# mynameisfiber/baton

Hardware: NVIDIA H100
Metric: federated local samples/sec (whole box), ResNet-18 FedAvg, synthetic non-IID 32x32 shards (higher is better)
Workload: dtype bf16

## Files before the change

baton_b200/csrc/bindings.cpp:

```cpp
#include <ATen/cuda/CUDAContext.h>
#include <c10/cuda/CUDAGuard.h>
#include <torch/extension.h>

#include <optional>
#include <vector>

#include "launch.h"

namespace {

inline cudaStream_t cur_stream() { return at::cuda::getCurrentCUDAStream().stream(); }
inline void check(int rc, const char* what) {
  TORCH_CHECK(rc == 0, "baton_b200::", what, " failed with code ", rc,
              rc > 0 ? std::string(" (") + cudaGetErrorString(static_cast<cudaError_t>(rc)) + ")" : std::string());
}
inline const void* cptr(const at::Tensor& t) { return t.data_ptr(); }
inline void* ptr(at::Tensor& t) { return t.data_ptr(); }
template <class T>
inline T* opt_ptr(const std::optional<at::Tensor>& t) {
  return (t.has_value() && t->defined()) ? reinterpret_cast<T*>(t->data_ptr()) : nullptr;
}
#define CHECK_CUDA(x) TORCH_CHECK((x).is_cuda(), #x " must be a CUDA tensor")

inline const float* prox_anchor(const std::optional<at::Tensor>& anchor, int64_t numel, const at::Tensor& hyper) {
// ... 233 lines not shown
  const int64_t c = src.size(3);
  const int64_t rows = src.size(0) * ((src.size(1) - 1) / stride + 1) * ((src.size(2) - 1) / stride + 1);
  TORCH_CHECK(rows > 0 && out.numel() % rows == 0, "conv_halo: out must hold [N*Ho*Wo, Nout] elements");
  const int64_t nout = out.numel() / rows;
  TORCH_CHECK(w.numel() == (dgrad ? c * 9 * nout : nout * 9 * c), "conv_halo: w must be [Cout, 9*Cin]");
  TORCH_CHECK(dgrad ? !col_stats.has_value()
                    : (!col_stats.has_value() || (col_stats->scalar_type() == at::kFloat && col_stats->numel() >= 2 * nout)),
              "conv_halo: col_stats is a [2 Cout] fp32 buffer of the forward");
  const c10::cuda::CUDAGuard guard(src.device());
  const int rc = b200_conv_halo(cptr(src), cptr(w), ptr(out), static_cast<int>(src.size(0)), static_cast<int>(src.size(1)),
                                static_cast<int>(src.size(2)), static_cast<int>(c), static_cast<int>(nout),
                                static_cast<int>(stride), dgrad ? 1 : 0, static_cast<int>(mc), opt_ptr<float>(col_stats),
                                cur_stream());
  if (rc == -2) return false;
  check(rc, "conv_halo");
  return true;
}
bool conv_igemm_dgrad_s2(const at::Tensor& dy, const at::Tensor& w, at::Tensor dx, int64_t kh, int64_t kw,
                         const std::vector<int64_t>& ntaps, const std::vector<int64_t>& taps, int64_t force_bn) {
  CHECK_CUDA(dy); CHECK_CUDA(w); CHECK_CUDA(dx);
  TORCH_CHECK(dy.scalar_type() == at::kBFloat16 && w.scalar_type() == at::kBFloat16 && dx.scalar_type() == at::kBFloat16 &&
              dy.dim() == 4 && dx.dim() == 4 && dy.is_contiguous() && w.is_contiguous() && dx.is_contiguous());
  TORCH_CHECK(ntaps.size() == 4 && taps.size() == 16, "conv_igemm_dgrad_s2: 4 classes x 4 taps");
  int nt[4], tw[16];
  for (int i = 0; i < 4; ++i) nt[i] = static_cast<int>(ntaps[i]);
  for (int i = 0; i < 16; ++i) tw[i] = static_cast<int>(taps[i]);
  const c10::cuda::CUDAGuard guard(dy.device());
  const int rc = b200_conv_igemm_dgrad_s2(cptr(dy), cptr(w), ptr(dx), static_cast<int>(dx.size(0)),
                                          static_cast<int>(dx.size(1)), static_cast<int>(dx.size(2)),
                                          static_cast<int>(dx.size(3)), static_cast<int>(dy.size(3)), static_cast<int>(kh),
// ... 1160 lines not shown
  m.doc() = "baton_b200 sm_90a kernels";
  m.attr("MAX_RANKS") = B200_MAX_RANKS;
  m.def("gemm", &gemm);
  m.def("trace_set", &trace_set);
  m.def("attention_fwd", &attention_fwd);
  m.def("attention_bwd", &attention_bwd);
  m.def("bn_bwd_cluster", &bn_bwd_cluster);
  m.def("gn_fwd", &gn_fwd);
  m.def("gn_bwd", &gn_bwd);
  m.def("im2col_tma_probe", &im2col_tma_probe);
  m.def("conv_igemm_fwd", &conv_igemm_fwd);
  m.def("conv_igemm_wgrad", &conv_igemm_wgrad);
  m.def("conv_igemm_dgrad", &conv_igemm_dgrad);
  m.def("conv_igemm_dgrad_s2", &conv_igemm_dgrad_s2);
  m.def("conv_halo", &conv_halo);
  m.def("gemm_batched", &gemm_batched);
  m.def("gemm_fp8", &gemm_fp8);
  m.def("quant_mx_rows", &quant_mx_rows);
  m.def("quant_mx_cols", &quant_mx_cols);
  m.def("fused_sgd", &fused_sgd);
  m.def("fused_sgd_segments", &fused_sgd_segments);
  m.def("grad_norm_clip", &grad_norm_clip);
  m.attr("GRAD_NORM_WORK_WORDS") = B200_GRAD_NORM_WORK_WORDS;
  m.def("weighted_sum", &weighted_sum);
  m.def("fold_client", &fold_client);
  m.def("scaffold_corr", &scaffold_corr);
  m.def("scaffold_dc", &scaffold_dc);
  m.def("cast", &cast);
  m.def("gather_rows", &gather_rows);
  m.def("gather_augment", &gather_augment);
// ... 59 lines not shown
```

baton_b200/csrc/conv_halo.cu:

```cuda
#define B200_TU_TAG 12
#include "ptx.cuh"
#include "epilogue.cuh"
#include "launch.h"
#include "pdl.cuh"

namespace b200 {

constexpr int HALO_BM = 64;
constexpr int HALO_BN = 64;
constexpr int HALO_TAPS = 9;
constexpr int HALO_THREADS = 256;
constexpr int HALO_CONSUMERS = 128;
constexpr int HALO_SLOT_BYTES = 64 * 64 * 2;
constexpr int HALO_PART_PITCH = HALO_BN + 4;
constexpr int HALO_MAX_SMEM = 227 * 1024;

struct HaloParams {
  int M, N;
  int Ho, Wo;
  __nv_bfloat16* D;
  float* col_stats;
  int ncol;
  int mc;
  int halo_bytes;
};

__host__ __device__ constexpr int halo_barriers(int k_tiles) { return (1 + k_tiles + 15) / 16 * 16; }

__host__ __device__ constexpr int halo_fixed_bytes(int k_tiles) {
  return k_tiles * HALO_SLOT_BYTES + halo_barriers(k_tiles) * 8 + 4 * HALO_BN * 4 + 1024;
}

template <bool DGRAD, int CB, int STRIDE>
__global__ void __launch_bounds__(HALO_THREADS, 1)
conv_halo_kernel(const __grid_constant__ CUtensorMap tmX, const __grid_constant__ CUtensorMap tmW, const HaloParams p) {
  constexpr int KT = HALO_TAPS * CB;
  extern __shared__ __align__(1024) uint8_t smem_raw[];
  uint8_t* smem = reinterpret_cast<uint8_t*>((reinterpret_cast<uintptr_t>(smem_raw) + 1023) & ~uintptr_t(1023));
  uint8_t* halo = smem;
  uint8_t* bslot = smem + CB * p.halo_bytes;
  uint64_t* bar = reinterpret_cast<uint64_t*>(bslot + KT * HALO_SLOT_BYTES);
  float* cstat = reinterpret_cast<float*>(bar + halo_barriers(KT));

  griddep_launch_dependents();
  const int warp = threadIdx.x >> 5;
  const int m0 = blockIdx.y * HALO_BM;
  const int n0 = blockIdx.x * HALO_BN;
  const int hw = p.Ho * p.Wo;
  const int hp = STRIDE * (p.Ho - 1) + 3, wp = STRIDE * (p.Wo - 1) + 3;

  if (warp == 0 && elect_one()) {
    tma_prefetch_desc(&tmX);
    tma_prefetch_desc(&tmW);
    for (int i = 0; i < 1 + KT; ++i) mbar_init(&bar[i], 1);
    fence_barrier_init();
  }
  __syncthreads();
  if (p.mc > 1) cluster_sync_all();
  griddep_wait();

  if (warp == 0) {
    if (elect_one()) {
      const int imgs = HALO_BM / hw;
      mbar_expect_tx(&bar[0], CB * imgs * hp * wp * 128);
#pragma unroll
      for (int cb = 0; cb < CB; ++cb) tma_load_4d(halo + cb * p.halo_bytes, &tmX, &bar[0], 64 * cb, -1, -1, m0 / hw);
      const int rows = 64 / p.mc;
      const int rank = p.mc > 1 ? static_cast<int>(cluster_ctarank()) : 0;
      const uint16_t mask = static_cast<uint16_t>((1u << p.mc) - 1);
#pragma unroll 1
      for (int kt = 0; kt < KT; ++kt) {
        const int tap = kt / CB, cb = kt - tap * CB;
        mbar_expect_tx(&bar[1 + kt], HALO_SLOT_BYTES);
        uint8_t* dst = bslot + kt * HALO_SLOT_BYTES + rank * rows * 128;
        const int c0 = DGRAD ? (HALO_TAPS - 1 - tap) * p.ncol + n0 : kt * 64;
        const int c1 = DGRAD ? cb * 64 + rank * rows : n0 + rank * rows;
        if (p.mc > 1)
          tma_load_2d_mc(dst, &tmW, &bar[1 + kt], c0, c1, mask);
        else
          tma_load_2d(dst, &tmW, &bar[1 + kt], c0, c1);
      }
    }
  } else if (warp >= 4) {
    const int ew = warp - 4;
    const int lane = static_cast<int>(lane_id());
    const int m = 16 * ew + (lane & 15);
    const int img = m / hw, rem = m - img * hw;
    const int oi = rem / p.Wo, oj = rem - oi * p.Wo;
    const int hrow0 = (img * hp + STRIDE * oi) * wp + STRIDE * oj;
    const uint32_t halo_a = smem_u32(halo);
    const int half = lane >> 4;
    auto load_a = [&](uint32_t (&a)[4][4], int kt) {
      const int tap = kt / CB, cb = kt - tap * CB;
      const int r = tap / 3, s = tap - 3 * r;
      const int hrow = hrow0 + r * wp + s;
      const uint32_t row_addr = halo_a + static_cast<uint32_t>(cb * p.halo_bytes + hrow * 128);
#pragma unroll
      for (int kk = 0; kk < 4; ++kk) ldmatrix_x4(a[kk], row_addr + ((((2 * kk + half) ^ hrow) & 7) << 4));
    };

    float acc[32];
#pragma unroll
    for (int j = 0; j < 32; ++j) acc[j] = 0.f;
    uint32_t a[2][4][4];
    mbar_wait(&bar[0], 0);
    load_a(a[0], 0);
#pragma unroll
    for (int kt = 0; kt < KT; ++kt) {
      mbar_wait(&bar[1 + kt], 0);
      const uint32_t sb = smem_u32(bslot + kt * HALO_SLOT_BYTES);
      wgmma_fence();
#pragma unroll
      for (int kk = 0; kk < 4; ++kk) {
        const uint64_t bd = DGRAD ? gmma_desc_sw128(sb + kk * 2048, 8192, 1024) : gmma_desc_sw128(sb + kk * 32, 16, 1024);
        wgmma_bf16_n64_rs<DGRAD ? 1 : 0>(acc, a[kt & 1][kk], bd, 1u);
      }
      wgmma_commit();
      if (kt + 1 < KT) {
        wgmma_wait<1>();
        load_a(a[(kt + 1) & 1], kt + 1);
      }
    }
    wgmma_wait<0>();
    wgmma_fence_operands(acc);
    if (threadIdx.x == 128) TRACE_POINT();

    named_bar_sync(1, HALO_CONSUMERS);
    float* part = reinterpret_cast<float*>(smem);
    wg_store_acc<HALO_BN>(acc, part, HALO_PART_PITCH, 0);
    named_bar_sync(1, HALO_CONSUMERS);
    const int q = ew & 1;
    const int c = (ew >> 1) * 32;
    const int lrow = q * 32 + lane;
    const int row = m0 + lrow;
    const int col0 = n0 + c;
    float* sstat = cstat + q * 2 * HALO_BN;
    const bool want_stats = p.col_stats != nullptr;
    if (col0 >= p.N) {
      if (want_stats) { sstat[c + lane] = 0.f; sstat[HALO_BN + c + lane] = 0.f; }
    } else {
      uint32_t r[32];
      acc_ld_row32(part + lrow * HALO_PART_PITCH + c, r);
      float v[32];
#pragma unroll
      for (int j = 0; j < 32; ++j) v[j] = __uint_as_float(r[j]);
      if (want_stats) stage_col_stats(sstat, HALO_BN, c, v);
      if (row < p.M) {
        __nv_bfloat16* d = p.D + static_cast<size_t>(row) * p.N + col0;
        if (col0 + 32 <= p.N && (p.N % 8) == 0) {
#pragma unroll
          for (int j = 0; j < 32; j += 8) {
            uint4 o;
            o.x = pack_bf16x2(v[j], v[j + 1]);
            o.y = pack_bf16x2(v[j + 2], v[j + 3]);
            o.z = pack_bf16x2(v[j + 4], v[j + 5]);
            o.w = pack_bf16x2(v[j + 6], v[j + 7]);
            *reinterpret_cast<uint4*>(d + j) = o;
          }
        } else {
          _Pragma("unroll") for (int j = 0; j < 32; ++j) if (col0 + j < p.N) d[j] = __float2bfloat16_rn(v[j]);
        }
      }
    }
    if (want_stats) {
      named_bar_sync(1, HALO_CONSUMERS);
      for (int i = threadIdx.x - 128; i < 2 * HALO_BN; i += HALO_CONSUMERS) {
        const int col = i < HALO_BN ? i : i - HALO_BN;
        if (n0 + col < p.N)
          atomicAdd(p.col_stats + (i < HALO_BN ? 0 : p.N) + n0 + col,
                    cstat[i] + cstat[2 * HALO_BN + i]);
      }
    }
  }
}

template <auto KERNEL>
static int launch_halo(const CUtensorMap& tx, const CUtensorMap& tw, const HaloParams& p, dim3 grid, int smem,
                       cudaStream_t stream) {
  static bool configured = false;
  if (!configured) {
    cudaError_t e = cudaFuncSetAttribute(KERNEL, cudaFuncAttributeMaxDynamicSharedMemorySize,
                                         HALO_MAX_SMEM);
    if (e != cudaSuccess) return static_cast<int>(e);
    configured = true;
  }
// ... 11 lines not shown
  }
  if (p.mc > 1) {
    attr[na].id = cudaLaunchAttributeClusterDimension;
    attr[na].val.clusterDim.x = 1;
    attr[na].val.clusterDim.y = p.mc;
    attr[na].val.clusterDim.z = 1;
    ++na;
  }
  cfg.attrs = attr;
  cfg.numAttrs = na;
  cudaError_t le = cudaLaunchKernelEx(&cfg, KERNEL, tx, tw, p);
  if (le != cudaSuccess) return static_cast<int>(le);
  return static_cast<int>(cudaGetLastError());
}

}

extern "C" int b200_encode_map2_bf16(void* map, const void* base, long long rows, long long cols, long long ld,
                                     int box_cols, int box_rows);
extern "C" int b200_encode_map4_box_bf16(void* map, const void* base, const long long* dims,
                                         const long long* stride_bytes, const int* box);

extern "C" int b200_conv_halo(const void* src, const void* w, void* out, int N, int H, int W, int C, int Nout,
                              int stride, int dgrad, int mc, float* col_stats, cudaStream_t stream) {
  using namespace b200;
  const bool s1c64 = stride == 1 && C == 64, s1c128 = stride == 1 && C == 128, s2c64 = stride == 2 && C == 64 && !dgrad;
  if (!s1c64 && !s1c128 && !s2c64) return -2;
  const int Ho = (H - 1) / stride + 1, Wo = (W - 1) / stride + 1;
  const long long M = static_cast<long long>(N) * Ho * Wo;
  if (M <= 0 || Nout <= 0) return 0;
  const int hw = Ho * Wo;
  const long long m_tiles = (M + HALO_BM - 1) / HALO_BM;
  const int hp = stride * (Ho - 1) + 3, wp = stride * (Wo - 1) + 3;
  if (H <= 0 || W <= 0 || HALO_BM % hw != 0 || hp > 256 || wp > 256 || M > (1ll << 30) || Nout % 8 != 0 ||
      (dgrad && Nout % 64 != 0) || (mc != 1 && mc != 2 && mc != 4 && mc != 8) || m_tiles % mc != 0 ||
      (reinterpret_cast<uintptr_t>(src) & 15) || (reinterpret_cast<uintptr_t>(w) & 15) ||
      (reinterpret_cast<uintptr_t>(out) & 15))
    return -2;
  const int imgs = HALO_BM / hw;
  const int cb = C / 64;
  const int halo_bytes = (imgs * hp * wp * 128 + 1023) / 1024 * 1024;
  const int smem = cb * halo_bytes + halo_fixed_bytes(HALO_TAPS * cb);
  if (smem > HALO_MAX_SMEM) return -2;
  CUtensorMap tx, tw;
  const long long dims[4] = {C, W, H, N};
  const long long strides[3] = {static_cast<long long>(C) * 2, static_cast<long long>(W) * C * 2,
                                static_cast<long long>(H) * W * C * 2};
  const int box[4] = {64, wp, hp, imgs};
  int rc = b200_encode_map4_box_bf16(&tx, src, dims, strides, box);
  if (rc) return rc;
  const long long wrows = dgrad ? C : Nout, wcols = dgrad ? 9ll * Nout : 9ll * C;
  rc = b200_encode_map2_bf16(&tw, w, wrows, wcols, wcols, 64, 64 / mc);
  if (rc) return rc;
  HaloParams p;
  p.M = static_cast<int>(M); p.N = Nout; p.Ho = Ho; p.Wo = Wo; p.D = reinterpret_cast<__nv_bfloat16*>(out);
  p.col_stats = col_stats; p.ncol = Nout; p.mc = mc; p.halo_bytes = halo_bytes;
  dim3 grid((Nout + HALO_BN - 1) / HALO_BN, static_cast<unsigned>(m_tiles), 1);
  if (s2c64) return launch_halo<conv_halo_kernel<false, 1, 2>>(tx, tw, p, grid, smem, stream);
  if (s1c64)
    return dgrad ? launch_halo<conv_halo_kernel<true, 1, 1>>(tx, tw, p, grid, smem, stream)
                 : launch_halo<conv_halo_kernel<false, 1, 1>>(tx, tw, p, grid, smem, stream);
  return dgrad ? launch_halo<conv_halo_kernel<true, 2, 1>>(tx, tw, p, grid, smem, stream)
               : launch_halo<conv_halo_kernel<false, 2, 1>>(tx, tw, p, grid, smem, stream);
}

B200_TRACE_REGISTER(conv_halo)
```

baton_b200/csrc/gemm_wgmma.cu:

```cuda
#define B200_TU_TAG 1
#include "ptx.cuh"
#include "epilogue.cuh"
#include "launch.h"
#include "pdl.cuh"
#include "sgd.cuh"

namespace b200 {

constexpr int BM = 128;
constexpr int BK = 64;
constexpr int WG_K = 16;
constexpr int GEMM_THREADS = 384;
constexpr int CONSUMER_WARPS = 8;
constexpr int CONSUMER_THREADS = 32 * CONSUMER_WARPS;
constexpr int MAX_STAGES = 8;
constexpr int S2_MAX_TAPS = 4;

struct GemmParams {
  int M, N, K;
  void* D;
  long long ldd;
  const float* bias;
  int out_fp32;
  int act;
// ... 962 lines not shown
    cudaFree(nullptr);
    ctx_bound = true;
  }
  static EncodeTiledFn fn = nullptr;
  if (fn == nullptr) {
    void* ptr = nullptr;
    cudaDriverEntryPointQueryResult qres;
    cudaError_t e = cudaGetDriverEntryPoint("cuTensorMapEncodeTiled", &ptr, cudaEnableDefault, &qres);
    if (e != cudaSuccess || qres != cudaDriverEntryPointSuccess || ptr == nullptr) return nullptr;
    fn = reinterpret_cast<EncodeTiledFn>(ptr);
  }
  return fn;
}

static int make_map(CUtensorMap* map, const void* base, long long rows, long long cols, long long ld, int box_cols,
                    int box_rows) {
  EncodeTiledFn fn = get_encode_fn();
  if (fn == nullptr) return -1;
  cuuint64_t gdim[2] = {static_cast<cuuint64_t>(cols), static_cast<cuuint64_t>(rows)};
  cuuint64_t gstr[1] = {static_cast<cuuint64_t>(ld) * 2};
  cuuint32_t box[2] = {static_cast<cuuint32_t>(box_cols), static_cast<cuuint32_t>(box_rows)};
  cuuint32_t estr[2] = {1, 1};
  CUresult r = fn(map, CU_TENSOR_MAP_DATA_TYPE_BFLOAT16, 2, const_cast<void*>(base), gdim, gstr, box, estr,
                  CU_TENSOR_MAP_INTERLEAVE_NONE, CU_TENSOR_MAP_SWIZZLE_128B, CU_TENSOR_MAP_L2_PROMOTION_L2_256B,
                  CU_TENSOR_MAP_FLOAT_OOB_FILL_NONE);
  return r == CUDA_SUCCESS ? 0 : static_cast<int>(r);
}

static int make_map4(CUtensorMap* map, const void* base, long long rows, long long cols, long long ld, long long inner,
                     long long s_inner, long long outer, long long s_outer, int box_cols, int box_rows) {
  EncodeTiledFn fn = get_encode_fn();
  if (fn == nullptr) return -1;
  cuuint64_t gdim[4] = {static_cast<cuuint64_t>(cols), static_cast<cuuint64_t>(rows), static_cast<cuuint64_t>(inner),
                        static_cast<cuuint64_t>(outer)};
  cuuint64_t gstr[3] = {static_cast<cuuint64_t>(ld) * 2, static_cast<cuuint64_t>(s_inner) * 2,
                        static_cast<cuuint64_t>(s_outer) * 2};
  cuuint32_t box[4] = {static_cast<cuuint32_t>(box_cols), static_cast<cuuint32_t>(box_rows), 1, 1};
  cuuint32_t estr[4] = {1, 1, 1, 1};
  CUresult r = fn(map, CU_TENSOR_MAP_DATA_TYPE_BFLOAT16, 4, const_cast<void*>(base), gdim, gstr, box, estr,
// ... 115 lines not shown
    ++na;
  }
  cfg.attrs = attr;
  cfg.numAttrs = na;
  cudaError_t le = p.cluster_k > 1 ? cudaLaunchKernelEx(&cfg, gemm_bf16_splitk_kernel<BN, true, CONV, AFFINE>, ta, tb, p)
                                   : cudaLaunchKernelEx(&cfg, gemm_bf16_splitk_kernel<BN, false, CONV, AFFINE>, ta, tb, p);
  if (le != cudaSuccess) return static_cast<int>(le);
  return static_cast<int>(cudaGetLastError());
}

}

extern "C" int b200_encode_map2_bf16(void* map, const void* base, long long rows, long long cols, long long ld,
                                     int box_cols, int box_rows) {
  return b200::make_map(reinterpret_cast<CUtensorMap*>(map), base, rows, cols, ld, box_cols, box_rows);
}
extern "C" int b200_encode_map4_bf16(void* map, const void* base, long long rows, long long cols, long long ld,
                                     long long inner, long long s_inner, long long outer, long long s_outer,
                                     int box_cols, int box_rows) {
  return b200::make_map4(reinterpret_cast<CUtensorMap*>(map), base, rows, cols, ld, inner, s_inner, outer, s_outer,
                         box_cols, box_rows);
}
extern "C" int b200_encode_map4_box_bf16(void* map, const void* base, const long long* dims, const long long* stride_bytes,
                                         const int* box) {
  b200::EncodeTiledFn fn = b200::get_encode_fn();
  if (fn == nullptr) return -1;
  cuuint64_t gdim[4], gstr[3];
  cuuint32_t bx[4], estr[4] = {1, 1, 1, 1};
  for (int i = 0; i < 4; ++i) {
    gdim[i] = static_cast<cuuint64_t>(dims[i]);
// ... 333 lines not shown
```

baton_b200/csrc/launch.h:

```cpp
#pragma once
#include <cuda_runtime.h>
#include <stdint.h>

#define B200_MAX_RANKS 16

extern "C" {

struct B200SgdEpilogue {
  float* theta;
  void* theta_bf16;
  float* mom;
  const float* hyper;
  int nesterov;
  const float* anchor;
  const float* corr;
  float* v;
};
#define B200_SGD_EPILOGUE_DECLINED (-6)

struct B200AffineEpilogue {
  const float* scale;
  const float* shift;
  const void* residual;
  long long ldr;
// ... 19 lines not shown
                            const B200Dropout* drop, cudaStream_t stream);
int b200_attention_drop_bwd(const void* qkv, const void* dout, const void* probs, void* dqkv, int B, int S, int H, int dh,
                            float scale, const B200Dropout* drop, cudaStream_t stream);
int b200_conv_igemm_fwd(const void* x, const void* w, void* y, int N, int H, int W, int Cin, int Cout, int KH, int KW,
                        int stride, int pad, int Ho, int Wo, int cluster_k, int force_bn, float* col_stats,
                        const B200AffineEpilogue* affine, cudaStream_t stream);
int b200_conv_igemm_dgrad(const void* dy, const void* w, void* dx, int N, int H, int W, int Cin, int Cout, int KH, int KW,
                          int pad, int Ho, int Wo, int cluster_k, int force_bn, cudaStream_t stream);
int b200_conv_igemm_dgrad_s2(const void* dy, const void* w, void* dx, int N, int H, int W, int Cin, int Cout, int KH,
                             int KW, int Ho, int Wo, const int* ntaps, const int* taps, int force_bn, cudaStream_t stream);
int b200_conv_igemm_wgrad(const void* dy, const void* x, float* dw, int N, int H, int W, int Cin, int Cout, int KH, int KW,
                          int stride, int pad, int Ho, int Wo, int split_k, int force_bn, const B200SgdEpilogue* sgd,
                          cudaStream_t stream);
int b200_conv_halo(const void* src, const void* w, void* out, int N, int H, int W, int C, int Nout, int stride,
                   int dgrad, int mc, float* col_stats, cudaStream_t stream);
int b200_im2col_tma_probe(const void* x, void* col, int N, int H, int W, int C, int KH, int KW, int stride, int pad,
                          int Ho, int Wo, cudaStream_t stream);
int b200_gemm_fp8(const void* a, const void* b, void* d, const float* bias, const void* sfa, const void* sfb, int M, int N,
                  int K, long long lda, long long ldb, long long ldd, int out_fp32, int act, int split_k, int accumulate,
                  float alpha, cudaStream_t stream);
int b200_quant_mx_rows(const void* x, void* q, void* sf, long long R, int C, long long ld_in, int Cp, cudaStream_t stream);
int b200_quant_mx_cols(const void* x, void* q, void* sf, long long R, int C, long long ld_in, long long Rp,
                       cudaStream_t stream);
int b200_gemm_simt(const void* a, const void* b, void* d, const float* bias, int M, int N, int K, long long lda,
                   long long ldb, long long ldd, int a_mn, int b_mn, int out_fp32, int act, int accumulate,
                   float alpha, cudaStream_t stream);

int b200_fused_sgd(float* w, float* g, float* mom, void* w_bf16, long long n, const float* hyper, int zero_grad,
                   int nesterov, const unsigned long long* wire_slot, const float* pack_global,
                   const float* pack_scale, long long n_pack, int wire_fp32, const float* prox_anchor,
// ... 240 lines not shown
```

baton_b200/csrc/ptx.cuh:

```cuda
#pragma once
#include <cuda.h>
#include <cuda_bf16.h>
#include <cuda_runtime.h>
#include <stdint.h>

namespace b200 {

__device__ __forceinline__ uint32_t smem_u32(const void* p) {
  return static_cast<uint32_t>(__cvta_generic_to_shared(p));
}
__device__ __forceinline__ uint32_t lane_id() {
  uint32_t l;
  asm volatile("mov.u32 %0, %%laneid;" : "=r"(l));
  return l;
}
__device__ __forceinline__ bool elect_one() {
  uint32_t pred;
  asm volatile(
      "{\n\t.reg .pred p;\n\t"
      "elect.sync _|p, 0xffffffff;\n\t"
      "selp.u32 %0, 1, 0, p;\n\t}"
      : "=r"(pred));
  return pred != 0;
}
// ... 78 lines not shown
}
template <int NR>
__device__ __forceinline__ void wgmma_fence_operands(float (&d)[NR]) {
#pragma unroll
  for (int i = 0; i < NR; ++i) asm volatile("" : "+f"(d[i])::"memory");
}

__device__ __forceinline__ uint64_t gmma_desc_sw128(uint32_t smem_addr, uint32_t lbo_bytes, uint32_t sbo_bytes) {
  uint64_t d = 0;
  d |= static_cast<uint64_t>((smem_addr & 0x3FFFF) >> 4);
  d |= static_cast<uint64_t>((lbo_bytes >> 4) & 0x3FFF) << 16;
  d |= static_cast<uint64_t>((sbo_bytes >> 4) & 0x3FFF) << 32;
  d |= static_cast<uint64_t>(1) << 62;
  return d;
}

template <int TA, int TB>
__device__ __forceinline__ void wgmma_bf16_n64(float (&d)[32], uint64_t da, uint64_t db, uint32_t scale_d) {
  asm volatile(
      "{\n\t.reg .pred p;\n\tsetp.ne.b32 p, %34, 0;\n\t"
      "wgmma.mma_async.sync.aligned.m64n64k16.f32.bf16.bf16 "
      "{"
      "%0, %1, %2, %3, %4, %5, %6, %7, %8, %9, %10, %11, %12, %13, %14, %15, "
      "%16, %17, %18, %19, %20, %21, %22, %23, %24, %25, %26, %27, %28, %29, %30, %31"
      "}, %32, %33, p, 1, 1, %35, %36;\n\t}"
      : "+f"(d[0]), "+f"(d[1]), "+f"(d[2]), "+f"(d[3]), "+f"(d[4]), "+f"(d[5]), "+f"(d[6]), "+f"(d[7]),
        "+f"(d[8]), "+f"(d[9]), "+f"(d[10]), "+f"(d[11]), "+f"(d[12]), "+f"(d[13]), "+f"(d[14]), "+f"(d[15]),
        "+f"(d[16]), "+f"(d[17]), "+f"(d[18]), "+f"(d[19]), "+f"(d[20]), "+f"(d[21]), "+f"(d[22]), "+f"(d[23]),
        "+f"(d[24]), "+f"(d[25]), "+f"(d[26]), "+f"(d[27]), "+f"(d[28]), "+f"(d[29]), "+f"(d[30]), "+f"(d[31])
      : "l"(da), "l"(db), "r"(scale_d), "n"(TA), "n"(TB));
// ... 20 lines not shown
      : "l"(da), "l"(db), "r"(scale_d), "n"(TA), "n"(TB));
}
template <int TB>
__device__ __forceinline__ void wgmma_bf16_n64_rs(float (&d)[32], const uint32_t (&a)[4], uint64_t db, uint32_t scale_d) {
  asm volatile(
      "{\n\t.reg .pred p;\n\tsetp.ne.b32 p, %37, 0;\n\t"
      "wgmma.mma_async.sync.aligned.m64n64k16.f32.bf16.bf16 "
      "{"
      "%0, %1, %2, %3, %4, %5, %6, %7, %8, %9, %10, %11, %12, %13, %14, %15, "
      "%16, %17, %18, %19, %20, %21, %22, %23, %24, %25, %26, %27, %28, %29, %30, %31"
      "}, {%32, %33, %34, %35}, %36, p, 1, 1, %38;\n\t}"
      : "+f"(d[0]), "+f"(d[1]), "+f"(d[2]), "+f"(d[3]), "+f"(d[4]), "+f"(d[5]), "+f"(d[6]), "+f"(d[7]),
        "+f"(d[8]), "+f"(d[9]), "+f"(d[10]), "+f"(d[11]), "+f"(d[12]), "+f"(d[13]), "+f"(d[14]), "+f"(d[15]),
        "+f"(d[16]), "+f"(d[17]), "+f"(d[18]), "+f"(d[19]), "+f"(d[20]), "+f"(d[21]), "+f"(d[22]), "+f"(d[23]),
        "+f"(d[24]), "+f"(d[25]), "+f"(d[26]), "+f"(d[27]), "+f"(d[28]), "+f"(d[29]), "+f"(d[30]), "+f"(d[31])
      : "r"(a[0]), "r"(a[1]), "r"(a[2]), "r"(a[3]), "l"(db), "r"(scale_d), "n"(TB));
}
__device__ __forceinline__ void ldmatrix_x4(uint32_t (&r)[4], uint32_t smem_addr) {
  asm volatile("ldmatrix.sync.aligned.m8n8.x4.shared.b16 {%0, %1, %2, %3}, [%4];"
               : "=r"(r[0]), "=r"(r[1]), "=r"(r[2]), "=r"(r[3])
               : "r"(smem_addr)
               : "memory");
}
__device__ __forceinline__ void wgmma_e4m3_n64(float (&d)[32], uint64_t da, uint64_t db, uint32_t scale_d) {
  asm volatile(
      "{\n\t.reg .pred p;\n\tsetp.ne.b32 p, %34, 0;\n\t"
      "wgmma.mma_async.sync.aligned.m64n64k32.f32.e4m3.e4m3 "
      "{"
      "%0, %1, %2, %3, %4, %5, %6, %7, %8, %9, %10, %11, %12, %13, %14, %15, "
      "%16, %17, %18, %19, %20, %21, %22, %23, %24, %25, %26, %27, %28, %29, %30, %31"
// ... 140 lines not shown
```

baton_b200/ops/functional.py:

```python
from __future__ import annotations

import collections
import functools
from typing import List, Optional, Sequence, Tuple

import torch

from ._ext import load

BF16 = torch.bfloat16
NUM_SMS = 132


def _pitch(t: torch.Tensor) -> int:
    assert t.dim() == 2 and (t.stride(1) == 1 or t.shape[1] == 1), "GEMM operand must have unit inner stride"
    return t.stride(0) if t.shape[0] > 1 else max(t.stride(0), t.shape[1])


def _tma_ok(t: torch.Tensor) -> bool:
    return t.dtype == BF16 and _pitch(t) % 8 == 0 and t.data_ptr() % 16 == 0


def pick_bn(M: int, N: int) -> int:
    m_tiles = (M + 127) // 128
# ... 412 lines not shown

def halo_eligible(kh: int, kw: int, stride: int, pad: int, c: int, h: int, w: int,
                  affine: Optional[dict] = None, dgrad: bool = False) -> bool:
    if kh != 3 or kw != 3 or pad != 1 or (stride, c) not in _HALO_FORMS or (dgrad and stride != 1):
        return False
    hw = conv_out_size(h, 3, stride, 1) * conv_out_size(w, 3, stride, 1)
    return (hw <= HALO_BM and HALO_BM % hw == 0 and affine is None and
            halo_smem_bytes(h, w, c, stride) <= _HALO_MAX_SMEM)


def halo_cluster(m_rows: int) -> int:
    tiles = (m_rows + HALO_BM - 1) // HALO_BM
    return 4 if tiles % 4 == 0 else 2 if tiles % 2 == 0 else 1


def _conv_path(path: Optional[str], eligible: bool) -> str:
    if path is None:
        return "halo" if eligible else "im2col"
    if path not in ("halo", "im2col"):
        raise ValueError("path must be None, 'halo' or 'im2col', not {!r}".format(path))
    if path == "halo" and not eligible:
        raise ValueError("the halo kernel does not take this convolution (see halo_eligible)")
    return path


def conv_igemm_fwd(x: torch.Tensor, w2d: torch.Tensor, kh: int, kw: int, stride: int, pad: int,
                   col_stats: Optional[torch.Tensor] = None, affine: Optional[dict] = None,
                   cluster_k: Optional[int] = None, force_bn: int = 0,
                   out: Optional[torch.Tensor] = None, path: Optional[str] = None,
                   mc: Optional[int] = None) -> Optional[torch.Tensor]:
    n, h, w, c = x.shape
    cout = w2d.shape[0]
    if c % 64 or w2d.shape[1] != kh * kw * c or not x.is_contiguous() or not w2d.is_contiguous():
        return None
    ho, wo = conv_out_size(h, kh, stride, pad), conv_out_size(w, kw, stride, pad)
    M, K = n * ho * wo, kh * kw * c
    halo = halo_eligible(kh, kw, stride, pad, c, h, w, affine) and cout % 8 == 0
    if _conv_path(path, halo) == "halo":
        y = out if out is not None else torch.empty((M, cout), dtype=BF16, device=x.device)
        if not load().conv_halo(x, w2d, y, stride, False, mc or halo_cluster(M), col_stats):
            raise RuntimeError("conv_halo declined a convolution halo_eligible admits")
        return y
    bn = force_bn or pick_bn(M, cout)
    if cluster_k is None:
        cluster_k = pick_cluster_k(M, cout, K, bn)
    y = out if out is not None else torch.empty((M, cout), dtype=BF16, device=x.device)
    af = affine or {}
    ok = load().conv_igemm_fwd(x, w2d, y, kh, kw, stride, pad, ho, wo, cluster_k, bn, col_stats, af.get("scale"),
                               af.get("shift"), af.get("residual"), bool(af.get("relu", False)))
    return y if ok else None


S2_MAX_TAPS = 4


def conv_s2_dgrad_taps(kh: int, kw: int, pad: int, ho: int, wo: int) -> Optional[List[List[Tuple[int, int, int]]]]:
# ... 14 lines not shown
                    if dp < ho and dq < wo:
                        taps.append((r * kw + s, dp, dq))
            if len(taps) > S2_MAX_TAPS:
                return None
            classes.append(taps)
    return classes


def conv_igemm_dgrad(dy: torch.Tensor, w2d: torch.Tensor, in_shape, kh: int, kw: int, pad: int, stride: int = 1,
                     out: Optional[torch.Tensor] = None, path: Optional[str] = None,
                     mc: Optional[int] = None, cluster_k: Optional[int] = None) -> Optional[torch.Tensor]:
    n, h, w, c = in_shape
    cout = dy.shape[-1]
    if c % 64 or cout % 64 or w2d.shape[1] != kh * kw * c or not dy.is_contiguous() or not w2d.is_contiguous():
        return None
    if _conv_path(path, halo_eligible(kh, kw, stride, pad, cout, h, w, dgrad=True)) == "halo":
        dx = out if out is not None else torch.empty((n, h, w, c), dtype=BF16, device=dy.device)
        if not load().conv_halo(dy, w2d, dx, 1, True, mc or halo_cluster(n * h * w), None):
            raise RuntimeError("conv_halo declined a convolution halo_eligible admits")
        return dx
    if stride == 1:
        M, K = n * h * w, kh * kw * cout
        bn = pick_bn(M, c)
        dx = out if out is not None else torch.empty((n, h, w, c), dtype=BF16, device=dy.device)
        if cluster_k is None:
            cluster_k = pick_cluster_k(M, c, K, bn)
        ok = load().conv_igemm_dgrad(dy, w2d, dx, kh, kw, pad, cluster_k, bn)
        return dx if ok else None
    if stride != 2:
        return None
    ho, wo = dy.shape[1], dy.shape[2]
    classes = conv_s2_dgrad_taps(kh, kw, pad, ho, wo)
    if classes is None:
        return None
# ... 220 lines not shown
```

Before: 223,900.

## Add small-feature-map conv kernel with whole-image tiles and 32-wide columns

Adds a conv_smallmap path for 3x3 pad-1 convolutions on small maps (stride-1 C=256 and stride-2 C=128), used in both forward and dgrad. The kernel stages whole images in shared memory with no TMA padding halo and reads a zero line in place of out-of-image taps. It uses n32 wgmma tiles with 64B-swizzled weight loads, which yields more CTAs on the deep ResNet layers, where M is small and the im2col GEMM path underfills the GPU. The cost is more kernel variants, extra per-tap bounds checks, and halved N per MMA.

```diff
diff --git a/baton_b200/csrc/bindings.cpp b/baton_b200/csrc/bindings.cpp
--- a/baton_b200/csrc/bindings.cpp
+++ b/baton_b200/csrc/bindings.cpp
@@ -271,6 +271,29 @@
                                 cur_stream());
   if (rc == -2) return false;
   check(rc, "conv_halo");
+  return true;
+}
+bool conv_smallmap(const at::Tensor& src, const at::Tensor& w, at::Tensor out, int64_t stride, bool dgrad, int64_t mc,
+                   int64_t bn, const std::optional<at::Tensor>& col_stats) {
+  CHECK_CUDA(src); CHECK_CUDA(w); CHECK_CUDA(out);
+  TORCH_CHECK(src.scalar_type() == at::kBFloat16 && w.scalar_type() == at::kBFloat16 && out.scalar_type() == at::kBFloat16 &&
+              src.dim() == 4 && src.is_contiguous() && w.is_contiguous() && out.is_contiguous());
+  TORCH_CHECK(stride == 1 || stride == 2, "conv_smallmap: stride 1 or 2");
+  const int64_t c = src.size(3);
+  const int64_t rows = src.size(0) * ((src.size(1) - 1) / stride + 1) * ((src.size(2) - 1) / stride + 1);
+  TORCH_CHECK(rows > 0 && out.numel() % rows == 0, "conv_smallmap: out must hold [N*Ho*Wo, Nout] elements");
+  const int64_t nout = out.numel() / rows;
+  TORCH_CHECK(w.numel() == (dgrad ? c * 9 * nout : nout * 9 * c), "conv_smallmap: w must be [Cout, 9*Cin]");
+  TORCH_CHECK(dgrad ? !col_stats.has_value()
+                    : (!col_stats.has_value() || (col_stats->scalar_type() == at::kFloat && col_stats->numel() >= 2 * nout)),
+              "conv_smallmap: col_stats is a [2 Cout] fp32 buffer of the forward");
+  const c10::cuda::CUDAGuard guard(src.device());
+  const int rc = b200_conv_smallmap(cptr(src), cptr(w), ptr(out), static_cast<int>(src.size(0)),
+                                    static_cast<int>(src.size(1)), static_cast<int>(src.size(2)), static_cast<int>(c),
+                                    static_cast<int>(nout), static_cast<int>(stride), dgrad ? 1 : 0, static_cast<int>(mc),
+                                    static_cast<int>(bn), opt_ptr<float>(col_stats), cur_stream());
+  if (rc == -2) return false;
+  check(rc, "conv_smallmap");
   return true;
 }
 bool conv_igemm_dgrad_s2(const at::Tensor& dy, const at::Tensor& w, at::Tensor dx, int64_t kh, int64_t kw,
@@ -1461,6 +1484,7 @@
   m.def("conv_igemm_dgrad", &conv_igemm_dgrad);
   m.def("conv_igemm_dgrad_s2", &conv_igemm_dgrad_s2);
   m.def("conv_halo", &conv_halo);
+  m.def("conv_smallmap", &conv_smallmap);
   m.def("gemm_batched", &gemm_batched);
   m.def("gemm_fp8", &gemm_fp8);
   m.def("quant_mx_rows", &quant_mx_rows);
diff --git a/baton_b200/csrc/conv_halo.cu b/baton_b200/csrc/conv_halo.cu
--- a/baton_b200/csrc/conv_halo.cu
+++ b/baton_b200/csrc/conv_halo.cu
@@ -11,9 +11,8 @@
 constexpr int HALO_TAPS = 9;
 constexpr int HALO_THREADS = 256;
 constexpr int HALO_CONSUMERS = 128;
-constexpr int HALO_SLOT_BYTES = 64 * 64 * 2;
-constexpr int HALO_PART_PITCH = HALO_BN + 4;
 constexpr int HALO_MAX_SMEM = 227 * 1024;
+constexpr int HALO_ZERO_BYTES = 128;
 
 struct HaloParams {
   int M, N;
@@ -23,31 +22,39 @@
   int ncol;
   int mc;
   int halo_bytes;
+  int bh, bw;
 };
 
 __host__ __device__ constexpr int halo_barriers(int k_tiles) { return (1 + k_tiles + 15) / 16 * 16; }
 
-__host__ __device__ constexpr int halo_fixed_bytes(int k_tiles) {
-  return k_tiles * HALO_SLOT_BYTES + halo_barriers(k_tiles) * 8 + 4 * HALO_BN * 4 + 1024;
-}
-
-template <bool DGRAD, int CB, int STRIDE>
+__host__ __device__ constexpr int halo_slot_bytes(int bn) { return bn * 64 * 2; }
+
+__host__ __device__ constexpr int halo_fixed_bytes(int k_tiles, int bn = HALO_BN, bool img = false) {
+  return k_tiles * halo_slot_bytes(bn) + halo_barriers(k_tiles) * 8 + 4 * bn * 4 + (img ? HALO_ZERO_BYTES : 0) + 1024;
+}
+
+template <bool DGRAD, int CB, int STRIDE, int BN = HALO_BN, bool IMG = false>
 __global__ void __launch_bounds__(HALO_THREADS, 1)
 conv_halo_kernel(const __grid_constant__ CUtensorMap tmX, const __grid_constant__ CUtensorMap tmW, const HaloParams p) {
+  static_assert(BN == 32 || BN == 64, "conv_halo_kernel: 32 or 64 columns");
   constexpr int KT = HALO_TAPS * CB;
+  constexpr int SLOT = halo_slot_bytes(BN);
+  constexpr int PITCH = BN + 4;
+  constexpr int ORIGIN = IMG ? 0 : -1;
   extern __shared__ __align__(1024) uint8_t smem_raw[];
   uint8_t* smem = reinterpret_cast<uint8_t*>((reinterpret_cast<uintptr_t>(smem_raw) + 1023) & ~uintptr_t(1023));
   uint8_t* halo = smem;
   uint8_t* bslot = smem + CB * p.halo_bytes;
-  uint64_t* bar = reinterpret_cast<uint64_t*>(bslot + KT * HALO_SLOT_BYTES);
+  uint64_t* bar = reinterpret_cast<uint64_t*>(bslot + KT * SLOT);
   float* cstat = reinterpret_cast<float*>(bar + halo_barriers(KT));
+  uint8_t* zline = reinterpret_cast<uint8_t*>(cstat + 4 * BN);
 
   griddep_launch_dependents();
   const int warp = threadIdx.x >> 5;
   const int m0 = blockIdx.y * HALO_BM;
-  const int n0 = blockIdx.x * HALO_BN;
+  const int n0 = blockIdx.x * BN;
   const int hw = p.Ho * p.Wo;
-  const int hp = STRIDE * (p.Ho - 1) + 3, wp = STRIDE * (p.Wo - 1) + 3;
+  const int hp = p.bh, wp = p.bw;
 
   if (warp == 0 && elect_one()) {
     tma_prefetch_desc(&tmX);
@@ -64,15 +71,19 @@
       const int imgs = HALO_BM / hw;
       mbar_expect_tx(&bar[0], CB * imgs * hp * wp * 128);
 #pragma unroll
-      for (int cb = 0; cb < CB; ++cb) tma_load_4d(halo + cb * p.halo_bytes, &tmX, &bar[0], 64 * cb, -1, -1, m0 / hw);
-      const int rows = 64 / p.mc;
+      for (int cb = 0; cb < CB; ++cb)
+        tma_load_4d(halo + cb * p.halo_bytes, &tmX, &bar[0], 64 * cb, ORIGIN, ORIGIN, m0 / hw);
+      constexpr int SROWS = DGRAD ? 64 : BN;
+      constexpr int RB = SLOT / SROWS;
+      const int rows = max(SROWS / p.mc, 8);
       const int rank = p.mc > 1 ? static_cast<int>(cluster_ctarank()) : 0;
       const uint16_t mask = static_cast<uint16_t>((1u << p.mc) - 1);
 #pragma unroll 1
       for (int kt = 0; kt < KT; ++kt) {
         const int tap = kt / CB, cb = kt - tap * CB;
-        mbar_expect_tx(&bar[1 + kt], HALO_SLOT_BYTES);
-        uint8_t* dst = bslot + kt * HALO_SLOT_BYTES + rank * rows * 128;
+        mbar_expect_tx(&bar[1 + kt], SLOT);
+        if (rank * rows >= SROWS) continue;
+        uint8_t* dst = bslot + kt * SLOT + rank * rows * RB;
         const int c0 = DGRAD ? (HALO_TAPS - 1 - tap) * p.ncol + n0 : kt * 64;
         const int c1 = DGRAD ? cb * 64 + rank * rows : n0 + rank * rows;
         if (p.mc > 1)
@@ -87,33 +98,53 @@
     const int m = 16 * ew + (lane & 15);
     const int img = m / hw, rem = m - img * hw;
     const int oi = rem / p.Wo, oj = rem - oi * p.Wo;
-    const int hrow0 = (img * hp + STRIDE * oi) * wp + STRIDE * oj;
+    const int y0 = STRIDE * oi - 1 - ORIGIN, x0 = STRIDE * oj - 1 - ORIGIN;
+    const int hrow0 = (img * hp + y0) * wp + x0;
     const uint32_t halo_a = smem_u32(halo);
     const int half = lane >> 4;
     auto load_a = [&](uint32_t (&a)[4][4], int kt) {
       const int tap = kt / CB, cb = kt - tap * CB;
       const int r = tap / 3, s = tap - 3 * r;
       const int hrow = hrow0 + r * wp + s;
-      const uint32_t row_addr = halo_a + static_cast<uint32_t>(cb * p.halo_bytes + hrow * 128);
+      uint32_t row_addr = halo_a + static_cast<uint32_t>(cb * p.halo_bytes + hrow * 128);
+      if constexpr (IMG) {
+        const int y = y0 + r, x = x0 + s;
+        if (y < 0 || y >= hp || x < 0 || x >= wp) row_addr = smem_u32(zline);
+      }
 #pragma unroll
       for (int kk = 0; kk < 4; ++kk) ldmatrix_x4(a[kk], row_addr + ((((2 * kk + half) ^ hrow) & 7) << 4));
     };
 
-    float acc[32];
-#pragma unroll
-    for (int j = 0; j < 32; ++j) acc[j] = 0.f;
+    float acc[BN / 2];
+#pragma unroll
+    for (int j = 0; j < BN / 2; ++j) acc[j] = 0.f;
     uint32_t a[2][4][4];
+    if constexpr (IMG) {
+      if (threadIdx.x < 128 + HALO_ZERO_BYTES / 16) reinterpret_cast<uint4*>(zline)[threadIdx.x - 128] = make_uint4(0, 0, 0, 0);
+      named_bar_sync(1, HALO_CONSUMERS);
+    }
     mbar_wait(&bar[0], 0);
+    if (threadIdx.x == 128) TRACE_POINT();
     load_a(a[0], 0);
 #pragma unroll
     for (int kt = 0; kt < KT; ++kt) {
       mbar_wait(&bar[1 + kt], 0);
-      const uint32_t sb = smem_u32(bslot + kt * HALO_SLOT_BYTES);
+      if (threadIdx.x == 128 && (kt == 0 || kt == KT - 1)) TRACE_POINT();
+      const uint32_t sb = smem_u32(bslot + kt * SLOT);
       wgmma_fence();
 #pragma unroll
       for (int kk = 0; kk < 4; ++kk) {
-        const uint64_t bd = DGRAD ? gmma_desc_sw128(sb + kk * 2048, 8192, 1024) : gmma_desc_sw128(sb + kk * 32, 16, 1024);
-        wgmma_bf16_n64_rs<DGRAD ? 1 : 0>(acc, a[kt & 1][kk], bd, 1u);
+        uint64_t bd;
+        if constexpr (!DGRAD)
+          bd = gmma_desc_sw128(sb + kk * 32, 16, 1024);
+        else if constexpr (BN == 64)
+          bd = gmma_desc_sw128(sb + kk * 2048, 8192, 1024);
+        else
+          bd = gmma_desc_sw64(sb + kk * 1024, 4096, 512);
+        if constexpr (BN == 64)
+          wgmma_bf16_n64_rs<DGRAD ? 1 : 0>(acc, a[kt & 1][kk], bd, 1u);
+        else
+          wgmma_bf16_n32_rs<DGRAD ? 1 : 0>(acc, a[kt & 1][kk], bd, 1u);
       }
       wgmma_commit();
       if (kt + 1 < KT) {
@@ -127,24 +158,25 @@
 
     named_bar_sync(1, HALO_CONSUMERS);
     float* part = reinterpret_cast<float*>(smem);
-    wg_store_acc<HALO_BN>(acc, part, HALO_PART_PITCH, 0);
+    wg_store_acc<BN>(acc, part, PITCH, 0);
     named_bar_sync(1, HALO_CONSUMERS);
     const int q = ew & 1;
     const int c = (ew >> 1) * 32;
     const int lrow = q * 32 + lane;
     const int row = m0 + lrow;
     const int col0 = n0 + c;
-    float* sstat = cstat + q * 2 * HALO_BN;
+    float* sstat = cstat + q * 2 * BN;
     const bool want_stats = p.col_stats != nullptr;
-    if (col0 >= p.N) {
-      if (want_stats) { sstat[c + lane] = 0.f; sstat[HALO_BN + c + lane] = 0.f; }
+    if (c >= BN) {
+    } else if (col0 >= p.N) {
+      if (want_stats) { sstat[c + lane] = 0.f; sstat[BN + c + lane] = 0.f; }
     } else {
       uint32_t r[32];
-      acc_ld_row32(part + lrow * HALO_PART_PITCH + c, r);
+      acc_ld_row32(part + lrow * PITCH + c, r);
       float v[32];
 #pragma unroll
       for (int j = 0; j < 32; ++j) v[j] = __uint_as_float(r[j]);
-      if (want_stats) stage_col_stats(sstat, HALO_BN, c, v);
+      if (want_stats) stage_col_stats(sstat, BN, c, v);
       if (row < p.M) {
         __nv_bfloat16* d = p.D + static_cast<size_t>(row) * p.N + col0;
         if (col0 + 32 <= p.N && (p.N % 8) == 0) {
@@ -164,11 +196,11 @@
     }
     if (want_stats) {
       named_bar_sync(1, HALO_CONSUMERS);
-      for (int i = threadIdx.x - 128; i < 2 * HALO_BN; i += HALO_CONSUMERS) {
-        const int col = i < HALO_BN ? i : i - HALO_BN;
+      for (int i = threadIdx.x - 128; i < 2 * BN; i += HALO_CONSUMERS) {
+        const int col = i < BN ? i : i - BN;
         if (n0 + col < p.N)
-          atomicAdd(p.col_stats + (i < HALO_BN ? 0 : p.N) + n0 + col,
-                    cstat[i] + cstat[2 * HALO_BN + i]);
+          atomicAdd(p.col_stats + (i < BN ? 0 : p.N) + n0 + col,
+                    cstat[i] + cstat[2 * BN + i]);
       }
     }
   }
@@ -210,48 +242,72 @@
   return static_cast<int>(cudaGetLastError());
 }
 
+static int conv_tiled_setup(const void* src, const void* w, void* out, int N, int H, int W, int C, int Nout, int stride,
+                            int dgrad, int mc, int bn, bool img, float* col_stats, CUtensorMap* tx, CUtensorMap* tw,
+                            HaloParams* p, dim3* grid, int* smem);
+
 }
 
 extern "C" int b200_encode_map2_bf16(void* map, const void* base, long long rows, long long cols, long long ld,
                                      int box_cols, int box_rows);
+extern "C" int b200_encode_map2_sw64_bf16(void* map, const void* base, long long rows, long long cols, long long ld,
+                                          int box_cols, int box_rows);
 extern "C" int b200_encode_map4_box_bf16(void* map, const void* base, const long long* dims,
                                          const long long* stride_bytes, const int* box);
+
+namespace b200 {
+
+static int conv_tiled_setup(const void* src, const void* w, void* out, int N, int H, int W, int C, int Nout, int stride,
+                            int dgrad, int mc, int bn, bool img, float* col_stats, CUtensorMap* tx, CUtensorMap* tw,
+                            HaloParams* p, dim3* grid, int* smem) {
+  const int Ho = (H - 1) / stride + 1, Wo = (W - 1) / stride + 1;
+  const long long M = static_cast<long long>(N) * Ho * Wo;
+  if (M <= 0 || Nout <= 0) return 1;
+  const int hw = Ho * Wo;
+  const long long m_tiles = (M + HALO_BM - 1) / HALO_BM;
+  const int bh = img ? H : stride * (Ho - 1) + 3, bw = img ? W : stride * (Wo - 1) + 3;
+  if (H <= 0 || W <= 0 || HALO_BM % hw != 0 || bh > 256 || bw > 256 || M > (1ll << 30) || Nout % 8 != 0 ||
+      ((dgrad || img) && Nout % bn != 0) || (mc != 1 && mc != 2 && mc != 4 && mc != 8) || m_tiles % mc != 0 ||
+      (reinterpret_cast<uintptr_t>(src) & 15) || (reinterpret_cast<uintptr_t>(w) & 15) ||
+      (reinterpret_cast<uintptr_t>(out) & 15))
+    return -2;
+  const int imgs = HALO_BM / hw;
+  const int cb = C / 64;
+  const int box_bytes = (imgs * bh * bw * 128 + 1023) / 1024 * 1024;
+  *smem = cb * box_bytes + halo_fixed_bytes(HALO_TAPS * cb, bn, img);
+  if (*smem > HALO_MAX_SMEM) return -2;
+  const long long dims[4] = {C, W, H, N};
+  const long long strides[3] = {static_cast<long long>(C) * 2, static_cast<long long>(W) * C * 2,
+                                static_cast<long long>(H) * W * C * 2};
+  const int box[4] = {64, bw, bh, imgs};
+  int rc = b200_encode_map4_box_bf16(tx, src, dims, strides, box);
+  if (rc) return rc;
+  const long long wrows = dgrad ? C : Nout, wcols = dgrad ? 9ll * Nout : 9ll * C;
+  const int srows = dgrad ? 64 : bn;
+  const int rows = srows / mc > 8 ? srows / mc : 8;
+  rc = dgrad && bn == 32 ? b200_encode_map2_sw64_bf16(tw, w, wrows, wcols, wcols, bn, rows)
+                         : b200_encode_map2_bf16(tw, w, wrows, wcols, wcols, dgrad ? bn : 64, rows);
+  if (rc) return rc;
+  p->M = static_cast<int>(M); p->N = Nout; p->Ho = Ho; p->Wo = Wo; p->D = reinterpret_cast<__nv_bfloat16*>(out);
+  p->col_stats = col_stats; p->ncol = Nout; p->mc = mc; p->halo_bytes = box_bytes; p->bh = bh; p->bw = bw;
+  *grid = dim3((Nout + bn - 1) / bn, static_cast<unsigned>(m_tiles), 1);
+  return 0;
+}
+
+}
 
 extern "C" int b200_conv_halo(const void* src, const void* w, void* out, int N, int H, int W, int C, int Nout,
                               int stride, int dgrad, int mc, float* col_stats, cudaStream_t stream) {
   using namespace b200;
   const bool s1c64 = stride == 1 && C == 64, s1c128 = stride == 1 && C == 128, s2c64 = stride == 2 && C == 64 && !dgrad;
   if (!s1c64 && !s1c128 && !s2c64) return -2;
-  const int Ho = (H - 1) / stride + 1, Wo = (W - 1) / stride + 1;
-  const long long M = static_cast<long long>(N) * Ho * Wo;
-  if (M <= 0 || Nout <= 0) return 0;
-  const int hw = Ho * Wo;
-  const long long m_tiles = (M + HALO_BM - 1) / HALO_BM;
-  const int hp = stride * (Ho - 1) + 3, wp = stride * (Wo - 1) + 3;
-  if (H <= 0 || W <= 0 || HALO_BM % hw != 0 || hp > 256 || wp > 256 || M > (1ll << 30) || Nout % 8 != 0 ||
-      (dgrad && Nout % 64 != 0) || (mc != 1 && mc != 2 && mc != 4 && mc != 8) || m_tiles % mc != 0 ||
-      (reinterpret_cast<uintptr_t>(src) & 15) || (reinterpret_cast<uintptr_t>(w) & 15) ||
-      (reinterpret_cast<uintptr_t>(out) & 15))
-    return -2;
-  const int imgs = HALO_BM / hw;
-  const int cb = C / 64;
-  const int halo_bytes = (imgs * hp * wp * 128 + 1023) / 1024 * 1024;
-  const int smem = cb * halo_bytes + halo_fixed_bytes(HALO_TAPS * cb);
-  if (smem > HALO_MAX_SMEM) return -2;
   CUtensorMap tx, tw;
-  const long long dims[4] = {C, W, H, N};
-  const long long strides[3] = {static_cast<long long>(C) * 2, static_cast<long long>(W) * C * 2,
-                                static_cast<long long>(H) * W * C * 2};
-  const int box[4] = {64, wp, hp, imgs};
-  int rc = b200_encode_map4_box_bf16(&tx, src, dims, strides, box);
-  if (rc) return rc;
-  const long long wrows = dgrad ? C : Nout, wcols = dgrad ? 9ll * Nout : 9ll * C;
-  rc = b200_encode_map2_bf16(&tw, w, wrows, wcols, wcols, 64, 64 / mc);
-  if (rc) return rc;
   HaloParams p;
-  p.M = static_cast<int>(M); p.N = Nout; p.Ho = Ho; p.Wo = Wo; p.D = reinterpret_cast<__nv_bfloat16*>(out);
-  p.col_stats = col_stats; p.ncol = Nout; p.mc = mc; p.halo_bytes = halo_bytes;
-  dim3 grid((Nout + HALO_BN - 1) / HALO_BN, static_cast<unsigned>(m_tiles), 1);
+  dim3 grid;
+  int smem = 0;
+  const int rc = conv_tiled_setup(src, w, out, N, H, W, C, Nout, stride, dgrad, mc, HALO_BN, false, col_stats, &tx, &tw,
+                                  &p, &grid, &smem);
+  if (rc) return rc == 1 ? 0 : rc;
   if (s2c64) return launch_halo<conv_halo_kernel<false, 1, 2>>(tx, tw, p, grid, smem, stream);
   if (s1c64)
     return dgrad ? launch_halo<conv_halo_kernel<true, 1, 1>>(tx, tw, p, grid, smem, stream)
@@ -260,4 +316,24 @@
                : launch_halo<conv_halo_kernel<false, 2, 1>>(tx, tw, p, grid, smem, stream);
 }
 
+extern "C" int b200_conv_smallmap(const void* src, const void* w, void* out, int N, int H, int W, int C, int Nout,
+                                  int stride, int dgrad, int mc, int bn, float* col_stats, cudaStream_t stream) {
+  using namespace b200;
+  const bool s1c256 = stride == 1 && C == 256 && bn == 32;
+  const bool s2c128 = stride == 2 && C == 128 && !dgrad && (bn == 32 || bn == 64);
+  if (!s1c256 && !s2c128) return -2;
+  CUtensorMap tx, tw;
+  HaloParams p;
+  dim3 grid;
+  int smem = 0;
+  const int rc = conv_tiled_setup(src, w, out, N, H, W, C, Nout, stride, dgrad, mc, bn, true, col_stats, &tx, &tw, &p,
+                                  &grid, &smem);
+  if (rc) return rc == 1 ? 0 : rc;
+  if (s2c128)
+    return bn == 32 ? launch_halo<conv_halo_kernel<false, 2, 2, 32, true>>(tx, tw, p, grid, smem, stream)
+                    : launch_halo<conv_halo_kernel<false, 2, 2, 64, true>>(tx, tw, p, grid, smem, stream);
+  return dgrad ? launch_halo<conv_halo_kernel<true, 4, 1, 32, true>>(tx, tw, p, grid, smem, stream)
+               : launch_halo<conv_halo_kernel<false, 4, 1, 32, true>>(tx, tw, p, grid, smem, stream);
+}
+
 B200_TRACE_REGISTER(conv_halo)
diff --git a/baton_b200/csrc/gemm_wgmma.cu b/baton_b200/csrc/gemm_wgmma.cu
--- a/baton_b200/csrc/gemm_wgmma.cu
+++ b/baton_b200/csrc/gemm_wgmma.cu
@@ -1000,7 +1000,7 @@
 }
 
 static int make_map(CUtensorMap* map, const void* base, long long rows, long long cols, long long ld, int box_cols,
-                    int box_rows) {
+                    int box_rows, CUtensorMapSwizzle swizzle = CU_TENSOR_MAP_SWIZZLE_128B) {
   EncodeTiledFn fn = get_encode_fn();
   if (fn == nullptr) return -1;
   cuuint64_t gdim[2] = {static_cast<cuuint64_t>(cols), static_cast<cuuint64_t>(rows)};
@@ -1008,7 +1008,7 @@
   cuuint32_t box[2] = {static_cast<cuuint32_t>(box_cols), static_cast<cuuint32_t>(box_rows)};
   cuuint32_t estr[2] = {1, 1};
   CUresult r = fn(map, CU_TENSOR_MAP_DATA_TYPE_BFLOAT16, 2, const_cast<void*>(base), gdim, gstr, box, estr,
-                  CU_TENSOR_MAP_INTERLEAVE_NONE, CU_TENSOR_MAP_SWIZZLE_128B, CU_TENSOR_MAP_L2_PROMOTION_L2_256B,
+                  CU_TENSOR_MAP_INTERLEAVE_NONE, swizzle, CU_TENSOR_MAP_L2_PROMOTION_L2_256B,
                   CU_TENSOR_MAP_FLOAT_OOB_FILL_NONE);
   return r == CUDA_SUCCESS ? 0 : static_cast<int>(r);
 }
@@ -1154,6 +1154,11 @@
 extern "C" int b200_encode_map2_bf16(void* map, const void* base, long long rows, long long cols, long long ld,
                                      int box_cols, int box_rows) {
   return b200::make_map(reinterpret_cast<CUtensorMap*>(map), base, rows, cols, ld, box_cols, box_rows);
+}
+extern "C" int b200_encode_map2_sw64_bf16(void* map, const void* base, long long rows, long long cols, long long ld,
+                                          int box_cols, int box_rows) {
+  return b200::make_map(reinterpret_cast<CUtensorMap*>(map), base, rows, cols, ld, box_cols, box_rows,
+                        CU_TENSOR_MAP_SWIZZLE_64B);
 }
 extern "C" int b200_encode_map4_bf16(void* map, const void* base, long long rows, long long cols, long long ld,
                                      long long inner, long long s_inner, long long outer, long long s_outer,
diff --git a/baton_b200/csrc/launch.h b/baton_b200/csrc/launch.h
--- a/baton_b200/csrc/launch.h
+++ b/baton_b200/csrc/launch.h
@@ -57,6 +57,8 @@
                           cudaStream_t stream);
 int b200_conv_halo(const void* src, const void* w, void* out, int N, int H, int W, int C, int Nout, int stride,
                    int dgrad, int mc, float* col_stats, cudaStream_t stream);
+int b200_conv_smallmap(const void* src, const void* w, void* out, int N, int H, int W, int C, int Nout, int stride,
+                       int dgrad, int mc, int bn, float* col_stats, cudaStream_t stream);
 int b200_im2col_tma_probe(const void* x, void* col, int N, int H, int W, int C, int KH, int KW, int stride, int pad,
                           int Ho, int Wo, cudaStream_t stream);
 int b200_gemm_fp8(const void* a, const void* b, void* d, const float* bias, const void* sfa, const void* sfb, int M, int N,
diff --git a/baton_b200/csrc/ptx.cuh b/baton_b200/csrc/ptx.cuh
--- a/baton_b200/csrc/ptx.cuh
+++ b/baton_b200/csrc/ptx.cuh
@@ -116,6 +116,14 @@
   d |= static_cast<uint64_t>(1) << 62;
   return d;
 }
+__device__ __forceinline__ uint64_t gmma_desc_sw64(uint32_t smem_addr, uint32_t lbo_bytes, uint32_t sbo_bytes) {
+  uint64_t d = 0;
+  d |= static_cast<uint64_t>((smem_addr & 0x3FFFF) >> 4);
+  d |= static_cast<uint64_t>((lbo_bytes >> 4) & 0x3FFF) << 16;
+  d |= static_cast<uint64_t>((sbo_bytes >> 4) & 0x3FFF) << 32;
+  d |= static_cast<uint64_t>(2) << 62;
+  return d;
+}
 
 template <int TA, int TB>
 __device__ __forceinline__ void wgmma_bf16_n64(float (&d)[32], uint64_t da, uint64_t db, uint32_t scale_d) {
@@ -166,6 +174,16 @@
         "+f"(d[8]), "+f"(d[9]), "+f"(d[10]), "+f"(d[11]), "+f"(d[12]), "+f"(d[13]), "+f"(d[14]), "+f"(d[15]),
         "+f"(d[16]), "+f"(d[17]), "+f"(d[18]), "+f"(d[19]), "+f"(d[20]), "+f"(d[21]), "+f"(d[22]), "+f"(d[23]),
         "+f"(d[24]), "+f"(d[25]), "+f"(d[26]), "+f"(d[27]), "+f"(d[28]), "+f"(d[29]), "+f"(d[30]), "+f"(d[31])
+      : "r"(a[0]), "r"(a[1]), "r"(a[2]), "r"(a[3]), "l"(db), "r"(scale_d), "n"(TB));
+}
+template <int TB>
+__device__ __forceinline__ void wgmma_bf16_n32_rs(float (&d)[16], const uint32_t (&a)[4], uint64_t db, uint32_t scale_d) {
+  asm volatile(
+      "{\n\t.reg .pred p;\n\tsetp.ne.b32 p, %21, 0;\n\t"
+      "wgmma.mma_async.sync.aligned.m64n32k16.f32.bf16.bf16 "
+      "{%0, %1, %2, %3, %4, %5, %6, %7, %8, %9, %10, %11, %12, %13, %14, %15}, {%16, %17, %18, %19}, %20, p, 1, 1, %22;\n\t}"
+      : "+f"(d[0]), "+f"(d[1]), "+f"(d[2]), "+f"(d[3]), "+f"(d[4]), "+f"(d[5]), "+f"(d[6]), "+f"(d[7]),
+        "+f"(d[8]), "+f"(d[9]), "+f"(d[10]), "+f"(d[11]), "+f"(d[12]), "+f"(d[13]), "+f"(d[14]), "+f"(d[15])
       : "r"(a[0]), "r"(a[1]), "r"(a[2]), "r"(a[3]), "l"(db), "r"(scale_d), "n"(TB));
 }
 __device__ __forceinline__ void ldmatrix_x4(uint32_t (&r)[4], uint32_t smem_addr) {
diff --git a/baton_b200/ops/functional.py b/baton_b200/ops/functional.py
--- a/baton_b200/ops/functional.py
+++ b/baton_b200/ops/functional.py
@@ -450,13 +450,36 @@
     return 4 if tiles % 4 == 0 else 2 if tiles % 2 == 0 else 1
 
 
-def _conv_path(path: Optional[str], eligible: bool) -> str:
+_SMALLMAP_FORMS = ((1, 256), (2, 128))
+SMALLMAP_BN = 32
+
+
+def smallmap_smem_bytes(h: int, w: int, c: int = 256, stride: int = 1, bn: int = SMALLMAP_BN) -> int:
+    ho, wo = conv_out_size(h, 3, stride, 1), conv_out_size(w, 3, stride, 1)
+    box = (HALO_BM // (ho * wo)) * h * w * 128
+    k_tiles = 9 * (c // 64)
+    return (c // 64 * round_up(box, 1024) + k_tiles * bn * 128 + round_up(1 + k_tiles, 16) * 8 + 4 * bn * 4 + 128
+            + 1024)
+
+
+def smallmap_eligible(kh: int, kw: int, stride: int, pad: int, c: int, h: int, w: int,
+                      affine: Optional[dict] = None, dgrad: bool = False) -> bool:
+    if kh != 3 or kw != 3 or pad != 1 or (stride, c) not in _SMALLMAP_FORMS or (dgrad and stride != 1):
+        return False
+    hw = conv_out_size(h, 3, stride, 1) * conv_out_size(w, 3, stride, 1)
+    return (hw <= HALO_BM and HALO_BM % hw == 0 and affine is None and
+            smallmap_smem_bytes(h, w, c, stride) <= _HALO_MAX_SMEM)
+
+
+def _conv_path(path: Optional[str], eligible: bool, smallmap: bool = False) -> str:
     if path is None:
-        return "halo" if eligible else "im2col"
-    if path not in ("halo", "im2col"):
-        raise ValueError("path must be None, 'halo' or 'im2col', not {!r}".format(path))
+        return "halo" if eligible else "smallmap" if smallmap else "im2col"
+    if path not in ("halo", "smallmap", "im2col"):
+        raise ValueError("path must be None, 'halo', 'smallmap' or 'im2col', not {!r}".format(path))
     if path == "halo" and not eligible:
         raise ValueError("the halo kernel does not take this convolution (see halo_eligible)")
+    if path == "smallmap" and not smallmap:
+        raise ValueError("the image-tile kernel does not take this convolution (see smallmap_eligible)")
     return path
 
 
@@ -464,7 +487,7 @@
                    col_stats: Optional[torch.Tensor] = None, affine: Optional[dict] = None,
                    cluster_k: Optional[int] = None, force_bn: int = 0,
                    out: Optional[torch.Tensor] = None, path: Optional[str] = None,
-                   mc: Optional[int] = None) -> Optional[torch.Tensor]:
+                   mc: Optional[int] = None, bn: int = SMALLMAP_BN) -> Optional[torch.Tensor]:
     n, h, w, c = x.shape
     cout = w2d.shape[0]
     if c % 64 or w2d.shape[1] != kh * kw * c or not x.is_contiguous() or not w2d.is_contiguous():
@@ -472,10 +495,17 @@
     ho, wo = conv_out_size(h, kh, stride, pad), conv_out_size(w, kw, stride, pad)
     M, K = n * ho * wo, kh * kw * c
     halo = halo_eligible(kh, kw, stride, pad, c, h, w, affine) and cout % 8 == 0
-    if _conv_path(path, halo) == "halo":
+    small = smallmap_eligible(kh, kw, stride, pad, c, h, w, affine) and cout % bn == 0
+    kind = _conv_path(path, halo, small)
+    if kind == "halo":
         y = out if out is not None else torch.empty((M, cout), dtype=BF16, device=x.device)
         if not load().conv_halo(x, w2d, y, stride, False, mc or halo_cluster(M), col_stats):
             raise RuntimeError("conv_halo declined a convolution halo_eligible admits")
+        return y
+    if kind == "smallmap":
+        y = out if out is not None else torch.empty((M, cout), dtype=BF16, device=x.device)
+        if not load().conv_smallmap(x, w2d, y, stride, False, mc or halo_cluster(M), bn, col_stats):
+            raise RuntimeError("conv_smallmap declined a convolution smallmap_eligible admits")
         return y
     bn = force_bn or pick_bn(M, cout)
     if cluster_k is None:
@@ -520,10 +550,17 @@
     cout = dy.shape[-1]
     if c % 64 or cout % 64 or w2d.shape[1] != kh * kw * c or not dy.is_contiguous() or not w2d.is_contiguous():
         return None
-    if _conv_path(path, halo_eligible(kh, kw, stride, pad, cout, h, w, dgrad=True)) == "halo":
+    kind = _conv_path(path, halo_eligible(kh, kw, stride, pad, cout, h, w, dgrad=True),
+                      smallmap_eligible(kh, kw, stride, pad, cout, h, w, dgrad=True) and c % SMALLMAP_BN == 0)
+    if kind == "halo":
         dx = out if out is not None else torch.empty((n, h, w, c), dtype=BF16, device=dy.device)
         if not load().conv_halo(dy, w2d, dx, 1, True, mc or halo_cluster(n * h * w), None):
             raise RuntimeError("conv_halo declined a convolution halo_eligible admits")
+        return dx
+    if kind == "smallmap":
+        dx = out if out is not None else torch.empty((n, h, w, c), dtype=BF16, device=dy.device)
+        if not load().conv_smallmap(dy, w2d, dx, 1, True, mc or halo_cluster(n * h * w), SMALLMAP_BN, None):
+            raise RuntimeError("conv_smallmap declined a convolution smallmap_eligible admits")
         return dx
     if stride == 1:
         M, K = n * h * w, kh * kw * cout
```

After: 230,600, median of 6. 1.03x the previous value.
